# KwonGihyun/TweedieMix

Measured on AMD Instinct MI355X. Metric: denoise steps/sec @ SDXL 1024^2 K=3 concepts (fusion phase); images/sec at 1/2/4/8 GPUs, higher is better.
Workload: dtype bf16

## Files before the change

### tweediemix_amd/csrc/gemm_convh.hip

```cpp
#include "gemm_kernel.h"

namespace tmix_gemm {

namespace {

constexpr int H_BN = 160, H_NS = 4, H_LW = 4, H_NW = 4;
constexpr int H_TR = 4, H_TC = 32;
constexpr int H_PC = H_TC + 2, H_PRV = (H_TR + 2) * H_PC;
constexpr int H_PI = 28;
constexpr int H_PATCH = 32 * 1024;
constexpr int H_WT = H_BN * 128;
constexpr int H_WI = H_BN / 8;
constexpr int H_OFF_W = 2 * H_PATCH;
constexpr int H_SA = 16 * 1024, H_LSA = 16 / H_LW;
constexpr int H_MAIN = H_OFF_W + H_NS * H_WT;
constexpr int H_LP = H_PI / H_LW, H_LWI = H_WI / H_LW;
constexpr int H_STG = 32 * (64 * 4 + 16);
static_assert(H_PI % H_LW == 0 && H_WI % H_LW == 0 && H_PI * 8 >= H_PRV && H_PI * 1024 <= H_PATCH - 4096, "loader geometry");
static_assert(2 * H_LWI + 2 * H_LSA <= 63 && 2 * H_LWI + H_LP <= 63, "vmcnt immediate");
static_assert(H_NW * H_STG <= H_NS * H_WT, "epilogue patches fit in the weight ring");

__global__ void __launch_bounds__((H_NW + H_LW) * 64, 2) conv_halo_kernel(const Params p) {
    extern __shared__ __attribute__((aligned(16))) char smem[];
    kernarg_touch<(int)sizeof(Params)>();
    const int tid = threadIdx.x, lane = tid & 63;
    const int w = __builtin_amdgcn_readfirstlane(tid >> 6);
    const bool loader = w >= H_NW;
    const bool prof_on = p.prof != nullptr && tid == 0;
    unsigned long long pt0 = 0, pt1 = 0, pt2 = 0;
    if (prof_on) pt0 = prof_enter(p.prof, (blockIdx.x | blockIdx.y) == 0, p.prof_detail);
    TMIX_PF_TOUCH(p, pf_keep, loader, H_LW * 64, tid - H_NW * 64);
    const TileId tile = tile_of_workgroup(p);
    const int tile_m = tile.tile_m, tile_n = tile.tile_n;
    const int n0 = tile_n * H_BN;
    const int txn = p.Wo / H_TC, tpi = (p.Ho / H_TR) * txn;
    const int img = tile_m / tpi, trem = tile_m - img * tpi;
    const int ty = trem / txn, tx = trem - ty * txn;
    const int y0 = ty * H_TR, x0 = tx * H_TC;
    const int nchunks = p.Cin / BK;
    const int n1 = p.S1 ? p.c1s / BK : 0, nsc = n1 + (p.S2 ? p.c2s / BK : 0);
    const int sa_base = ((nchunks - 1) & 1) ? 0 : H_PATCH;

    if (loader) {
        const __amdgpu_buffer_rsrc_t rsA = __builtin_amdgcn_make_buffer_rsrc((void*)p.A, 0, p.bytesA, 0x00020000);
        const __amdgpu_buffer_rsrc_t rsW = __builtin_amdgcn_make_buffer_rsrc((void*)p.W, 0, p.bytesW, 0x00020000);
        const int s = w - H_NW, lrow = lane >> 3;
        unsigned poff[H_LP], woff[H_LWI];
#pragma unroll
        for (int r = 0; r < H_LP; ++r) {
            const int row = (r * H_LW + s) * 8 + lrow;
            const int py = row / H_PC, px = row - py * H_PC;
            const int iy = y0 + py - 1, ix = x0 + px - 1;
            const bool ok = (row < H_PRV) & (iy >= 0) & (iy < p.H) & (ix >= 0) & (ix < p.Wd);
            const unsigned sw = (unsigned)(((lane & 7) ^ ((row >> 1) & 7)) * 16);
            poff[r] = ok ? (unsigned)((img * p.H + iy) * p.Wd + ix) * (unsigned)p.Cin * 2u + sw : 0x80000000u;
        }
#pragma unroll
        for (int r = 0; r < H_LWI; ++r) {
            const int row = (r * H_LW + s) * 8 + lrow;
            const unsigned sw = (unsigned)(((lane & 7) ^ ((row >> 1) & 7)) * 16);
            woff[r] = (unsigned)(n0 + row) * (unsigned)p.ldw * 2u + sw;
        }
        int spix[H_LSA]; unsigned ssw[H_LSA];
#pragma unroll
        for (int r = 0; r < H_LSA; ++r) {
            const int row = (r * H_LW + s) * 8 + lrow;
            spix[r] = (img * p.H + y0 + (row >> 5)) * p.Wd + x0 + (row & 31);
            ssw[r] = (unsigned)(((lane & 7) ^ ((row >> 1) & 7)) * 16);
        }
        auto stage_sa = [&](int j) __attribute__((always_inline)) {
            char* dst = smem + ((sa_base + (j % 3) * H_SA) & (2 * H_PATCH - 1));
            const bool first = j < n1;
            const __amdgpu_buffer_rsrc_t rs = __builtin_amdgcn_make_buffer_rsrc((void*)(first ? p.S1 : p.S2), 0, first ? p.bytesS1 : p.bytesS2, 0x00020000);
            const unsigned cs2 = (unsigned)(first ? p.c1s : p.c2s) * 2u, so = (unsigned)(first ? j : j - n1) * (BK * 2u);
#pragma unroll
            for (int r = 0; r < H_LSA; ++r) blds16(rs, j < nsc ? (unsigned)spix[r] * cs2 + ssw[r] : 0x80000000u, so, dst + (r * H_LW + s) * 1024);
        };
        auto stage_p = [&](int buf, int c, bool real) __attribute__((always_inline)) {
            char* dst = smem + buf * H_PATCH;
#pragma unroll
            for (int r = 0; r < H_LP; ++r) blds16(rsA, real ? poff[r] : 0x80000000u, (unsigned)c * (BK * 2), dst + (r * H_LW + s) * 1024);
        };
        auto stage_w = [&](int slot, int c, int t) __attribute__((always_inline)) {
            char* dst = smem + H_OFF_W + slot * H_WT;
            const unsigned so = c < nchunks ? (unsigned)(t * p.Cin + c * BK) * 2u : (unsigned)(9 * p.Cin + t * BK) * 2u;
#pragma unroll
            for (int r = 0; r < H_LWI; ++r) blds16(rsW, woff[r], so, dst + (r * H_LW + s) * 1024);
        };
        const int nk = nchunks * 9 + nsc;
        stage_p(0, 0, true);
        stage_w(0, 0, 0);
        stage_w(1, 0, 1);
        wait_vmcnt<H_LWI>();
        pf_keep_alive(pf_keep);
        __builtin_amdgcn_s_barrier();
        stage_w(2, 0, 2);
        int c3 = 0, t3 = 3, slot3 = 3;
        for (int c = 0; c < nchunks; ++c) {
#pragma unroll
            for (int t = 0; t < 9; ++t) {
                const int kt = c * 9 + t;
                const bool more = kt + 3 < nk;
                const bool sc_next = nsc > 0 && c == nchunks - 1;
                if (more) stage_w(slot3, c3, t3);
                if (t == 0) { if (sc_next) { stage_sa(0); stage_sa(1); } else stage_p((c + 1) & 1, c + 1, c + 1 < nchunks); }
                if (more) { if (t <= 2) { if (sc_next) wait_vmcnt<2 * H_LWI + 2 * H_LSA>(); else wait_vmcnt<2 * H_LWI + H_LP>(); } else wait_vmcnt<2 * H_LWI>(); }
                else wait_vmcnt<0>();
                __builtin_amdgcn_s_barrier();
                slot3 = (slot3 + 1) & 3;
                if (c3 < nchunks) { if (++t3 == 9) { t3 = 0; ++c3; } } else ++t3;
            }
        }
        for (int j = 0; j < nsc; ++j) {
            const bool more_w = j + 3 < nsc, more_a = j + 2 < nsc;
            if (more_w) stage_w(slot3, c3, t3);
            if (more_a) stage_sa(j + 2);
            if (more_w) wait_vmcnt<H_LWI + H_LSA>(); else if (more_a) wait_vmcnt<H_LSA>(); else wait_vmcnt<0>();
            __builtin_amdgcn_s_barrier();
            slot3 = (slot3 + 1) & 3;
            ++t3;
        }
        return;
    }

    const int l31 = lane & 31, lhi = lane >> 5;
    float* bias_lds = (float*)(smem + H_MAIN);
    float* rgb_lds = bias_lds + H_BN;
    if (tid < H_BN) {
        bias_lds[tid] = p.bias ? p.bias[n0 + tid] : 0.f;
        const int64_t m_first = (int64_t)img * p.Ho * p.Wo;
        rgb_lds[tid] = p.rgb ? p.rgb[(m_first / p.rows_per_group) * p.N + n0 + tid] : 0.f;
    }
    f32x16 acc[5];
#pragma unroll
    for (int j = 0; j < 5; ++j)
#pragma unroll
        for (int r = 0; r < 16; ++r) acc[j][r] = 0.f;

    int ppv = w * H_PC + l31;
    auto rd_a = [&](int buf, int t, int kk) __attribute__((always_inline)) -> frag_ab {
        const int pp = ppv + (t / 3) * H_PC + (t % 3);
        return *(const frag_ab*)(smem + buf * H_PATCH + pp * 128 + ((((kk * 2) + lhi) ^ ((pp >> 1) & 7)) << 4));
    };
    const int fsw = (lane >> 1) & 7;
    const int offW = H_OFF_W + l31 * 128;
    auto rd_b = [&](int slot, int j, int kk) __attribute__((always_inline)) -> frag_ab {
        return *(const frag_ab*)(smem + offW + slot * H_WT + j * 32 * 128 + ((((kk * 2) + lhi) ^ fsw) << 4));
    };
    const int64_t mrow0 = ((int64_t)img * p.Ho + y0 + w) * p.Wo + x0;
    uint4 rw[10];
    auto epi_prefetch = [&]() __attribute__((always_inline)) {
#pragma unroll
        for (int q = 0; q < 10; ++q) rw[q] = make_uint4(0u, 0u, 0u, 0u);
        if (p.R) {
#pragma unroll
            for (int c = 0; c < 2; ++c)
#pragma unroll
                for (int ps = 0; ps < 4; ++ps)
                    rw[c * 4 + ps] = *(const uint4*)(p.R + (mrow0 + ps * 8 + (lane >> 3)) * p.ldr + n0 + c * 64 + (lane & 7) * 8);
#pragma unroll
            for (int ps = 0; ps < 2; ++ps)
                rw[8 + ps] = *(const uint4*)(p.R + (mrow0 + ps * 16 + (lane >> 2)) * p.ldr + n0 + 128 + (lane & 3) * 8);
        }
    };

    __builtin_amdgcn_s_barrier();
    asm volatile("" ::: "memory");
    if (prof_on) pt1 = prof_now();
    frag_ab fa[2], fb[2][5];
    fa[0] = rd_a(0, 0, 0);
#pragma unroll
    for (int j = 0; j < 5; ++j) fb[0][j] = rd_b(0, j, 0);
    auto kstep = [&](const int S, const int nb, const int nt, const int ns, const int nkk) __attribute__((always_inline)) {
#pragma unroll
        for (int j = 0; j < 5; ++j) {
            acc[j] = __builtin_amdgcn_mfma_f32_32x32x16_bf16(fb[S][j], fa[S], acc[j], 0, 0, 0);
            __builtin_amdgcn_sched_barrier(0);
            if (j == 0) { fa[1 - S] = rd_a(nb, nt, nkk); fb[1 - S][0] = rd_b(ns, 0, nkk); }
            else if (j == 1) { fb[1 - S][1] = rd_b(ns, 1, nkk); fb[1 - S][2] = rd_b(ns, 2, nkk); }
            else if (j == 2) { fb[1 - S][3] = rd_b(ns, 3, nkk); fb[1 - S][4] = rd_b(ns, 4, nkk); }
            __builtin_amdgcn_sched_barrier(0);
        }
    };
    int cur = 0;
    for (int c = 0; c < nchunks; ++c) {
        const int buf = c & 1;
#pragma unroll
        for (int t = 0; t < 9; ++t) {
            if (t == 8 && c == nchunks - 1) { epi_prefetch(); __builtin_amdgcn_sched_barrier(0); }
            asm volatile("" : "+v"(ppv));
            kstep(0, buf, t, cur, 1);
            kstep(1, buf, t, cur, 2);
            kstep(0, buf, t, cur, 3);
            asm volatile("s_waitcnt lgkmcnt(0)" ::: "memory");
            __builtin_amdgcn_sched_barrier(0);
            __builtin_amdgcn_s_barrier();
            __builtin_amdgcn_sched_barrier(0);
            asm volatile("" ::: "memory");
            cur = (cur + 1) & 3;
            kstep(1, t == 8 ? (buf ^ 1) : buf, t == 8 ? 0 : t + 1, cur, 0);
        }
    }
    if (nsc > 0) {
        const int offS = (w * 32 + l31) * 128;
        auto rd_as = [&](int j, int kk) __attribute__((always_inline)) -> frag_ab {
            return *(const frag_ab*)(smem + ((sa_base + (j % 3) * H_SA) & (2 * H_PATCH - 1)) + offS + ((((kk * 2) + lhi) ^ fsw) << 4));
        };
        auto kstep_s = [&](const int S, const int nj, const int ns, const int nkk) __attribute__((always_inline)) {
#pragma unroll
            for (int j = 0; j < 5; ++j) {
                acc[j] = __builtin_amdgcn_mfma_f32_32x32x16_bf16(fb[S][j], fa[S], acc[j], 0, 0, 0);
                __builtin_amdgcn_sched_barrier(0);
                if (j == 0) { fa[1 - S] = rd_as(nj, nkk); fb[1 - S][0] = rd_b(ns, 0, nkk); }
                else if (j == 1) { fb[1 - S][1] = rd_b(ns, 1, nkk); fb[1 - S][2] = rd_b(ns, 2, nkk); }
                else if (j == 2) { fb[1 - S][3] = rd_b(ns, 3, nkk); fb[1 - S][4] = rd_b(ns, 4, nkk); }
                __builtin_amdgcn_sched_barrier(0);
            }
        };
        fa[0] = rd_as(0, 0);
        for (int j = 0; j < nsc; ++j) {
            kstep_s(0, j, cur, 1);
            kstep_s(1, j, cur, 2);
            kstep_s(0, j, cur, 3);
            asm volatile("s_waitcnt lgkmcnt(0)" ::: "memory");
            __builtin_amdgcn_sched_barrier(0);
            __builtin_amdgcn_s_barrier();
            __builtin_amdgcn_sched_barrier(0);
            asm volatile("" ::: "memory");
            cur = (cur + 1) & 3;
            kstep_s(1, j + 1, cur, 0);
        }
    }
    if (prof_on) pt2 = prof_now();

    char* stg = smem + H_OFF_W + w * H_STG;
    const int64_t blk = mrow0 >> 5;
    auto chunk = [&](int j0, auto cf_tag) __attribute__((always_inline)) {
        constexpr int CF = decltype(cf_tag)::value, CW = CF * 32, SR = CW * 4 + 16, LPR = CW / 8, RPI = 64 / LPR, NP = 32 / RPI;
        const int rr = lane / LPR, cc = (lane % LPR) * 8;
        const int nl = j0 * 32 + cc, nc = n0 + nl;
        const float4 bq0 = *(const float4*)(bias_lds + nl), bq1 = *(const float4*)(bias_lds + nl + 4);
        const float4 t0 = *(const float4*)(rgb_lds + nl), t1 = *(const float4*)(rgb_lds + nl + 4);
        const float bq[8] = {bq0.x, bq0.y, bq0.z, bq0.w, bq1.x, bq1.y, bq1.z, bq1.w};
        const float tq[8] = {t0.x, t0.y, t0.z, t0.w, t1.x, t1.y, t1.z, t1.w};
        float cv[16];
#pragma unroll
        for (int k = 0; k < 16; ++k) cv[k] = 0.f;
#pragma unroll
        for (int jj = 0; jj < CF; ++jj)
#pragma unroll
            for (int g = 0; g < 4; ++g)
                *(float4*)(stg + l31 * SR + (jj * 32 + g * 8 + lhi * 4) * 4) =
                    make_float4(acc[j0 + jj][g * 4 + 0], acc[j0 + jj][g * 4 + 1], acc[j0 + jj][g * 4 + 2], acc[j0 + jj][g * 4 + 3]);
#pragma unroll
        for (int ps = 0; ps < NP; ++ps) {
            const int r = ps * RPI + rr;
            const float4 v0 = *(const float4*)(stg + r * SR + cc * 4), v1 = *(const float4*)(stg + r * SR + cc * 4 + 16);
            float o[8] = {v0.x, v0.y, v0.z, v0.w, v1.x, v1.y, v1.z, v1.w};
#pragma unroll
            for (int k = 0; k < 8; ++k) o[k] = fmaf(o[k], 1.f, bq[k]) + tq[k];
            const uint4 rq = rw[(CF == 2 ? (j0 / 2) * 4 : 8) + ps];
            const unsigned ru[4] = {rq.x, rq.y, rq.z, rq.w};
#pragma unroll
            for (int k = 0; k < 4; ++k) { o[2 * k] += __uint_as_float(ru[k] << 16); o[2 * k + 1] += __uint_as_float(ru[k] & 0xffff0000u); }
            uint4 v;
            v.x = pack_bf2(o[0], o[1]); v.y = pack_bf2(o[2], o[3]); v.z = pack_bf2(o[4], o[5]); v.w = pack_bf2(o[6], o[7]);
            *(uint4*)(p.C + (mrow0 + r) * p.ldc + nc) = v;
            if (p.cs_out) {
                const unsigned u[4] = {v.x, v.y, v.z, v.w};
#pragma unroll
                for (int k = 0; k < 4; ++k) {
                    const float lo = __uint_as_float(u[k] << 16), hi = __uint_as_float(u[k] & 0xffff0000u);
                    cv[2 * k] += lo; cv[2 * k + 1] += hi;
                    cv[8 + 2 * k] = fmaf(lo, lo, cv[8 + 2 * k]); cv[9 + 2 * k] = fmaf(hi, hi, cv[9 + 2 * k]);
                }
            }
        }
        if (p.cs_out) {
            float tt[8], u[4];
#pragma unroll
            for (int k = 0; k < 8; ++k) tt[k] = swap32_sum(cv[k], cv[8 + k]);
#pragma unroll
            for (int k = 0; k < 4; ++k) u[k] = swap16_sum(tt[k], tt[k + 4]);
#pragma unroll
            for (int k = 0; k < 4; ++k) u[k] += dpp_row<0x128>(u[k]);
            if constexpr (CF == 1) {
#pragma unroll
                for (int k = 0; k < 4; ++k) u[k] += dpp_row<0x124>(u[k]);
            }
            if (!(lane & (CF == 1 ? 12 : 8)))
                *(float4*)(p.cs_out + (blk * 2 + (lane >> 5)) * p.N + nc + ((lane >> 4) & 1) * 4) = make_float4(u[0], u[1], u[2], u[3]);
        }
    };
    chunk(0, std::integral_constant<int, 2>{});
    chunk(2, std::integral_constant<int, 2>{});
    chunk(4, std::integral_constant<int, 1>{});
    if (prof_on) prof_leave(p.prof, p.prof_detail, pt0, pt1, pt2);
}

}

bool convh_eligible(const Params& p, int conv, int f8) {
    return conv && !f8 && p.mode == TMIX_CONV_S1 && p.ntaps == 9 && !p.scaleA && (p.wide & 1) && (p.Wo % H_TC) == 0 && (p.Ho % H_TR) == 0 && (p.N % H_BN) == 0
           && (p.Cin % BK) == 0 && (!p.rgb || p.rows_per_group % (p.Ho * p.Wo) == 0) && (!p.R || ((p.ldr % 8) == 0 && aligned16(p.R)));
}

int launch_convh(Params& p, hipStream_t st) {
    constexpr int SMEM = H_MAIN + 2 * H_BN * 4;
    static_assert(SMEM <= 160 * 1024, "LDS");
    p.tiles_m = p.M / 128; p.tiles_n = p.N / H_BN;
    p.group_m = 8;
    return launch_tiles<conv_halo_kernel>(p, p, 1, (H_NW + H_LW) * 64, SMEM, H_LW * 64, st, "conv3x3 (tiling 26)");
}

}
```

Measured before the change: 32.81.

## Switch conv-halo GEMM from 32x32x16 to 16x16x32 MFMA with register ring for weights

Replaces the 32x32x16 bf16 MFMA tiling with 16x16x32 MFMAs, giving two 16-row halves times ten 16-column fragments per warp. Weight fragments are streamed through a 5-entry register ring with a lag of three steps, and the trailing MFMAs of one tap are overlapped with the barrier hand-off into the next. Lane-to-row mapping is permuted (lp) so LDS reads stay conflict-free and the epilogue staging matches the new accumulator layout. This aims for finer-grained overlap of LDS reads and MFMA issue. The costs are more MFMA instructions per tile, a different register footprint, and a more intricate schedule.

```diff
diff --git a/tweediemix_amd/csrc/gemm_convh.hip b/tweediemix_amd/csrc/gemm_convh.hip
--- a/tweediemix_amd/csrc/gemm_convh.hip
+++ b/tweediemix_amd/csrc/gemm_convh.hip
@@ -123,7 +123,8 @@
         return;
     }
 
-    const int l31 = lane & 31, lhi = lane >> 5;
+    const int l15 = lane & 15, lq = lane >> 4;
+    const int lp = l15 < 4 ? 2 * l15 : (l15 < 12 ? 2 * l15 - 7 : 2 * l15 - 16);
     float* bias_lds = (float*)(smem + H_MAIN);
     float* rgb_lds = bias_lds + H_BN;
     if (tid < H_BN) {
@@ -131,21 +132,21 @@
         const int64_t m_first = (int64_t)img * p.Ho * p.Wo;
         rgb_lds[tid] = p.rgb ? p.rgb[(m_first / p.rows_per_group) * p.N + n0 + tid] : 0.f;
     }
-    f32x16 acc[5];
-#pragma unroll
-    for (int j = 0; j < 5; ++j)
-#pragma unroll
-        for (int r = 0; r < 16; ++r) acc[j][r] = 0.f;
-
-    int ppv = w * H_PC + l31;
-    auto rd_a = [&](int buf, int t, int kk) __attribute__((always_inline)) -> frag_ab {
-        const int pp = ppv + (t / 3) * H_PC + (t % 3);
-        return *(const frag_ab*)(smem + buf * H_PATCH + pp * 128 + ((((kk * 2) + lhi) ^ ((pp >> 1) & 7)) << 4));
+    f32x4 acc[2][10];
+#pragma unroll
+    for (int h = 0; h < 2; ++h)
+#pragma unroll
+        for (int j = 0; j < 10; ++j) acc[h][j] = (f32x4){0.f, 0.f, 0.f, 0.f};
+
+    int ppv = w * H_PC + lp;
+    auto rd_a = [&](int buf, int t, int ks, int h) __attribute__((always_inline)) -> frag_ab {
+        const int pp = ppv + (t / 3) * H_PC + (t % 3) + h * 16;
+        return *(const frag_ab*)(smem + buf * H_PATCH + pp * 128 + ((((ks * 4) + lq) ^ ((pp >> 1) & 7)) << 4));
     };
     const int fsw = (lane >> 1) & 7;
-    const int offW = H_OFF_W + l31 * 128;
-    auto rd_b = [&](int slot, int j, int kk) __attribute__((always_inline)) -> frag_ab {
-        return *(const frag_ab*)(smem + offW + slot * H_WT + j * 32 * 128 + ((((kk * 2) + lhi) ^ fsw) << 4));
+    const int offW = H_OFF_W + l15 * 128;
+    auto rd_b = [&](int slot, int m) __attribute__((always_inline)) -> frag_ab {
+        return *(const frag_ab*)(smem + offW + slot * H_WT + (m % 10) * 16 * 128 + (((((m / 10) * 4) + lq) ^ fsw) << 4));
     };
     const int64_t mrow0 = ((int64_t)img * p.Ho + y0 + w) * p.Wo + x0;
     uint4 rw[10];
@@ -164,71 +165,73 @@
         }
     };
 
+    constexpr int H_RW = 5, H_LAG = 3;
+    static_assert(20 % H_RW == 0 && H_LAG + 2 == H_RW, "W ring: step m + 20 must reuse the registers of step m, and the slot a read refills must just have been freed");
+    frag_ab fa[2][2], fb[H_RW];
+    auto mm = [&](const int m) __attribute__((always_inline)) {
+        acc[0][m % 10] = __builtin_amdgcn_mfma_f32_16x16x32_bf16(fb[m % H_RW], fa[m / 10][0], acc[0][m % 10], 0, 0, 0);
+        acc[1][m % 10] = __builtin_amdgcn_mfma_f32_16x16x32_bf16(fb[m % H_RW], fa[m / 10][1], acc[1][m % 10], 0, 0, 0);
+    };
+    auto head = [&](auto rda, const int slot, auto prev_tag) __attribute__((always_inline)) {
+        constexpr bool PREV = decltype(prev_tag)::value;
+        fa[0][0] = rda(0, 0); fa[0][1] = rda(0, 1);
+        fb[0] = rd_b(slot, 0); fb[1] = rd_b(slot, 1);
+        __builtin_amdgcn_sched_barrier(0);
+#pragma unroll
+        for (int q = 0; q < H_LAG; ++q) {
+            if constexpr (PREV) { mm(20 - H_LAG + q); __builtin_amdgcn_sched_barrier(0); }
+            fb[(q + 2) % H_RW] = rd_b(slot, q + 2);
+            __builtin_amdgcn_sched_barrier(0);
+        }
+    };
+    auto body = [&](auto rda, const int slot) __attribute__((always_inline)) {
+#pragma unroll
+        for (int q = H_LAG; q < 20; ++q) {
+            mm(q - H_LAG);
+            __builtin_amdgcn_sched_barrier(0);
+            if (q + 2 < 20) fb[(q + 2) % H_RW] = rd_b(slot, q + 2);
+            if (q == 6) fa[1][0] = rda(1, 0);
+            if (q == 7) fa[1][1] = rda(1, 1);
+            __builtin_amdgcn_sched_barrier(0);
+        }
+    };
+    auto hand_over = [&]() __attribute__((always_inline)) {
+        asm volatile("s_waitcnt lgkmcnt(0)" ::: "memory");
+        __builtin_amdgcn_sched_barrier(0);
+        __builtin_amdgcn_s_barrier();
+        __builtin_amdgcn_sched_barrier(0);
+        asm volatile("" ::: "memory");
+    };
+
     __builtin_amdgcn_s_barrier();
     asm volatile("" ::: "memory");
     if (prof_on) pt1 = prof_now();
-    frag_ab fa[2], fb[2][5];
-    fa[0] = rd_a(0, 0, 0);
-#pragma unroll
-    for (int j = 0; j < 5; ++j) fb[0][j] = rd_b(0, j, 0);
-    auto kstep = [&](const int S, const int nb, const int nt, const int ns, const int nkk) __attribute__((always_inline)) {
-#pragma unroll
-        for (int j = 0; j < 5; ++j) {
-            acc[j] = __builtin_amdgcn_mfma_f32_32x32x16_bf16(fb[S][j], fa[S], acc[j], 0, 0, 0);
-            __builtin_amdgcn_sched_barrier(0);
-            if (j == 0) { fa[1 - S] = rd_a(nb, nt, nkk); fb[1 - S][0] = rd_b(ns, 0, nkk); }
-            else if (j == 1) { fb[1 - S][1] = rd_b(ns, 1, nkk); fb[1 - S][2] = rd_b(ns, 2, nkk); }
-            else if (j == 2) { fb[1 - S][3] = rd_b(ns, 3, nkk); fb[1 - S][4] = rd_b(ns, 4, nkk); }
-            __builtin_amdgcn_sched_barrier(0);
-        }
-    };
     int cur = 0;
+    head([&](int ks, int h) __attribute__((always_inline)) { return rd_a(0, 0, ks, h); }, 0, std::false_type{});
     for (int c = 0; c < nchunks; ++c) {
         const int buf = c & 1;
 #pragma unroll
         for (int t = 0; t < 9; ++t) {
             if (t == 8 && c == nchunks - 1) { epi_prefetch(); __builtin_amdgcn_sched_barrier(0); }
             asm volatile("" : "+v"(ppv));
-            kstep(0, buf, t, cur, 1);
-            kstep(1, buf, t, cur, 2);
-            kstep(0, buf, t, cur, 3);
-            asm volatile("s_waitcnt lgkmcnt(0)" ::: "memory");
-            __builtin_amdgcn_sched_barrier(0);
-            __builtin_amdgcn_s_barrier();
-            __builtin_amdgcn_sched_barrier(0);
-            asm volatile("" ::: "memory");
+            body([&](int ks, int h) __attribute__((always_inline)) { return rd_a(buf, t, ks, h); }, cur);
+            hand_over();
             cur = (cur + 1) & 3;
-            kstep(1, t == 8 ? (buf ^ 1) : buf, t == 8 ? 0 : t + 1, cur, 0);
+            head([&](int ks, int h) __attribute__((always_inline)) { return rd_a(t == 8 ? (buf ^ 1) : buf, t == 8 ? 0 : t + 1, ks, h); }, cur, std::true_type{});
         }
     }
     if (nsc > 0) {
-        const int offS = (w * 32 + l31) * 128;
-        auto rd_as = [&](int j, int kk) __attribute__((always_inline)) -> frag_ab {
-            return *(const frag_ab*)(smem + ((sa_base + (j % 3) * H_SA) & (2 * H_PATCH - 1)) + offS + ((((kk * 2) + lhi) ^ fsw) << 4));
+        const int offS = (w * 32 + lp) * 128, fswa = (lp >> 1) & 7;
+        auto rd_as = [&](int j, int ks, int h) __attribute__((always_inline)) -> frag_ab {
+            return *(const frag_ab*)(smem + ((sa_base + (j % 3) * H_SA) & (2 * H_PATCH - 1)) + offS + h * 16 * 128 + ((((ks * 4) + lq) ^ fswa) << 4));
         };
-        auto kstep_s = [&](const int S, const int nj, const int ns, const int nkk) __attribute__((always_inline)) {
-#pragma unroll
-            for (int j = 0; j < 5; ++j) {
-                acc[j] = __builtin_amdgcn_mfma_f32_32x32x16_bf16(fb[S][j], fa[S], acc[j], 0, 0, 0);
-                __builtin_amdgcn_sched_barrier(0);
-                if (j == 0) { fa[1 - S] = rd_as(nj, nkk); fb[1 - S][0] = rd_b(ns, 0, nkk); }
-                else if (j == 1) { fb[1 - S][1] = rd_b(ns, 1, nkk); fb[1 - S][2] = rd_b(ns, 2, nkk); }
-                else if (j == 2) { fb[1 - S][3] = rd_b(ns, 3, nkk); fb[1 - S][4] = rd_b(ns, 4, nkk); }
-                __builtin_amdgcn_sched_barrier(0);
-            }
-        };
-        fa[0] = rd_as(0, 0);
+        fa[0][0] = rd_as(0, 0, 0); fa[0][1] = rd_as(0, 0, 1);
+        __builtin_amdgcn_sched_barrier(0);
         for (int j = 0; j < nsc; ++j) {
-            kstep_s(0, j, cur, 1);
-            kstep_s(1, j, cur, 2);
-            kstep_s(0, j, cur, 3);
-            asm volatile("s_waitcnt lgkmcnt(0)" ::: "memory");
-            __builtin_amdgcn_sched_barrier(0);
-            __builtin_amdgcn_s_barrier();
-            __builtin_amdgcn_sched_barrier(0);
-            asm volatile("" ::: "memory");
+            body([&](int ks, int h) __attribute__((always_inline)) { return rd_as(j, ks, h); }, cur);
+            hand_over();
             cur = (cur + 1) & 3;
-            kstep_s(1, j + 1, cur, 0);
+            head([&](int ks, int h) __attribute__((always_inline)) { return rd_as(j + 1, ks, h); }, cur, std::true_type{});
         }
     }
     if (prof_on) pt2 = prof_now();
@@ -247,11 +250,10 @@
 #pragma unroll
         for (int k = 0; k < 16; ++k) cv[k] = 0.f;
 #pragma unroll
-        for (int jj = 0; jj < CF; ++jj)
-#pragma unroll
-            for (int g = 0; g < 4; ++g)
-                *(float4*)(stg + l31 * SR + (jj * 32 + g * 8 + lhi * 4) * 4) =
-                    make_float4(acc[j0 + jj][g * 4 + 0], acc[j0 + jj][g * 4 + 1], acc[j0 + jj][g * 4 + 2], acc[j0 + jj][g * 4 + 3]);
+        for (int jf = 0; jf < 2 * CF; ++jf)
+#pragma unroll
+            for (int h = 0; h < 2; ++h)
+                *(f32x4*)(stg + (h * 16 + lp) * SR + (jf * 16 + lq * 4) * 4) = acc[h][2 * j0 + jf];
 #pragma unroll
         for (int ps = 0; ps < NP; ++ps) {
             const int r = ps * RPI + rr;
```

After: 33.04 (median of 6 runs). Within noise of the previous version (+0.7%).
